# fabrizioromanelli/ORBSLAM2

Hardware: AMD Instinct MI355X
Metric: frames/sec ORB extract+match, KITTI 1241×376 stereo, 2000 feats; 1/2/4/8 GPU (higher is better)
Workload: dtype u8; 1 GPU; Stereo-KITTI00-02 1241x376, 2000 features, 8 levels: extract L+R + ComputeStereoMatches (64 pairs per step per GPU, weak scaling); distinct_pairs=16, chains_in_flight=1, stream_groups=1, quadtree_kernel=3, parallelism=frame-pair sharding, no data-path collective

## Files before the change

orbslam2_amd/csrc/orbfe_common.hpp:

```cpp
#pragma once

#include "orbfe_device.h"
#include <cstdlib>

typedef short pk16 __attribute__((ext_vector_type(2)));
#define ORBFE_RSRC_FLAGS 0x00020000

__device__ __forceinline__ int lane_id() { return threadIdx.x & 63; }

__device__ __forceinline__ int row_sum_i32(int v)
{
    v += __builtin_amdgcn_update_dpp(0, v, 0xB1, 0xf, 0xf, true);
    v += __builtin_amdgcn_update_dpp(0, v, 0x4E, 0xf, 0xf, true);
    v += __builtin_amdgcn_update_dpp(0, v, 0x141, 0xf, 0xf, true);
    v += __builtin_amdgcn_update_dpp(0, v, 0x140, 0xf, 0xf, true);
    return v;
}
__device__ __forceinline__ int wave_sum_i32(int v)
{
    v = row_sum_i32(v);
    v += __builtin_amdgcn_update_dpp(0, v, 0x142, 0xa, 0xf, false);
    v += __builtin_amdgcn_update_dpp(0, v, 0x143, 0xc, 0xf, false);
    return __builtin_amdgcn_readlane(v, 63);
}
__device__ __forceinline__ unsigned wave_min_u32(unsigned v)
{
#pragma unroll
    for (int o = 32; o > 0; o >>= 1) {
        unsigned t = (unsigned)__shfl_xor((int)v, o, 64);
        v = t < v ? t : v;
    }
    return v;
}

__host__ __device__ __forceinline__ int xcd_split_log2(int n_units) { return n_units >= 5 ? 0 : n_units >= 3 ? 1 : n_units == 2 ? 2 : 3; }
__host__ __forceinline__ int xcd_grid(int blocks_per_unit, int n_units)
{
    const int lg = xcd_split_log2(n_units), per_xcd = (blocks_per_unit + (1 << lg) - 1) >> lg, side = 8 >> lg;
    return per_xcd * ((n_units + side - 1) / side) * 8;
}
__device__ __forceinline__ int small_div(int a, int b) { return (int)(((float)a + 0.5f) * __builtin_amdgcn_rcpf((float)b)); }
__device__ __forceinline__ bool xcd_map_of(int bid, int blocks_per_unit, int n_units, int &unit, int &blk);
__device__ __forceinline__ bool xcd_map(int blocks_per_unit, int n_units, int &unit, int &blk) { return xcd_map_of((int)blockIdx.x, blocks_per_unit, n_units, unit, blk); }
__device__ __forceinline__ bool xcd_map_of(int bid, int blocks_per_unit, int n_units, int &unit, int &blk)
{
    const int lg = xcd_split_log2(n_units), xcd = bid & 7, jb = bid >> 3;
    const int per_xcd = (blocks_per_unit + (1 << lg) - 1) >> lg;
    const int round = small_div(jb, per_xcd);
    unit = round * (8 >> lg) + (xcd >> lg);
    blk = ((jb - round * per_xcd) << lg) + (xcd & ((1 << lg) - 1));
    return unit < n_units && blk < blocks_per_unit;
}

__host__ __forceinline__ uint32_t xcd_map_magic_host(int blocks_per_unit, int n_units)
{
    const int lg = xcd_split_log2(n_units), per_xcd = (blocks_per_unit + (1 << lg) - 1) >> lg, side = 8 >> lg;
    const unsigned long long rounds = (unsigned long long)((n_units + side - 1) / side);
    if (per_xcd <= 1 || (unsigned long long)per_xcd * rounds * (unsigned long long)per_xcd >= (1ull << 32)) return 0u;
    return (uint32_t)(((1ull << 32) + (unsigned long long)per_xcd - 1ull) / (unsigned long long)per_xcd);
}
__device__ __forceinline__ bool xcd_map_of_magic(int bid, int blocks_per_unit, int n_units, uint32_t magic, int &unit, int &blk)
{
    if (magic == 0u) return xcd_map_of(bid, blocks_per_unit, n_units, unit, blk);
    const int lg = xcd_split_log2(n_units), xcd = bid & 7, jb = bid >> 3;
    const int per_xcd = (blocks_per_unit + (1 << lg) - 1) >> lg;
    const int round = (int)__builtin_amdgcn_readfirstlane((int)(((unsigned long long)(unsigned)jb * (unsigned long long)magic) >> 32));
    unit = round * (8 >> lg) + (xcd >> lg);
    blk = ((jb - round * per_xcd) << lg) + (xcd & ((1 << lg) - 1));
    return unit < n_units && blk < blocks_per_unit;
}

__device__ __forceinline__ bool xcd_map_magic(int blocks_per_unit, int n_units, uint32_t magic, int &unit, int &blk) { return xcd_map_of_magic((int)blockIdx.x, blocks_per_unit, n_units, magic, unit, blk); }

__device__ __forceinline__ int reflect101(int p, int len)
{
    if (len == 1) return 0;
    while (p < 0 || p >= len) {
        if (p < 0) p = -p;
        else p = 2 * len - 2 - p;
    }
    return p;
}

__device__ inline int block_excl_scan(const int *src, int *dst, int n, int *s_tmp)
{
    const int nt = blockDim.x, tid = threadIdx.x;
    const int per = (n + nt - 1) / nt;
    const int b = tid * per;
    const int e = (b + per < n) ? b + per : n;
    int sum = 0;
    for (int i = b; i < e; i++) sum += src[i];
    s_tmp[tid] = sum;
    __syncthreads();
    for (int off = 1; off < nt; off <<= 1) {
        int v = tid >= off ? s_tmp[tid - off] : 0;
        __syncthreads();
        s_tmp[tid] += v;
        __syncthreads();
    }
    const int total = s_tmp[nt - 1];
    int run = s_tmp[tid] - sum;
    for (int i = b; i < e; i++) {
        int v = src[i];
        dst[i] = run;
        run += v;
    }
    __syncthreads();
    return total;
}

__device__ __forceinline__ float fast_atan2_deg(float y, float x)
{
    const float p1 = __uint_as_float(0x4265226fu);
    const float p3 = __uint_as_float(0xc19556eeu);
    const float p5 = __uint_as_float(0x410e9fbfu);
    const float p7 = __uint_as_float(0xc0228ad9u);
    const float eps = 2.220446049250313e-16f;
    float ax = fabsf(x), ay = fabsf(y);
    float a, c, c2;
    if (ax >= ay) {
        c = __fdiv_rn(ay, __fadd_rn(ax, eps));
        c2 = __fmul_rn(c, c);
        a = __fmul_rn(__fadd_rn(__fmul_rn(__fadd_rn(__fmul_rn(__fadd_rn(__fmul_rn(p7, c2), p5), c2), p3), c2), p1), c);
    } else {
        c = __fdiv_rn(ax, __fadd_rn(ay, eps));
        c2 = __fmul_rn(c, c);
        a = __fsub_rn(90.f, __fmul_rn(__fadd_rn(__fmul_rn(__fadd_rn(__fmul_rn(__fadd_rn(__fmul_rn(p7, c2), p5), c2), p3), c2), p1), c));
    }
    if (x < 0) a = __fsub_rn(180.f, a);
    if (y < 0) a = __fsub_rn(360.f, a);
    return a;
}

__device__ __forceinline__ void sincos_det(float rad, float *s, float *c)
{
    const double TWO_OVER_PI = 6.36619772367581382433e-01;
    const double PIO2_HI = 1.57079632673412561417e+00;
    const double PIO2_LO = 6.07710050650619224932e-11;
    const double S1 = -1.66666666666666324348e-01, S2 = 8.33333333332248946124e-03,
                 S3 = -1.98412698298579493134e-04, S4 = 2.75573137070700676789e-06,
                 S5 = -2.50507602534068634195e-08, S6 = 1.58969099521155010221e-10;
    const double C1 = 4.16666666666666019037e-02, C2 = -1.38888888888741095749e-03,
                 C3 = 2.48015872894767294178e-05, C4 = -2.75573143513906633035e-07,
                 C5 = 2.08757232129817482790e-09, C6 = -1.13596475577881948265e-11;
    double x = (double)rad;
    double t = __dadd_rn(__dmul_rn(x, TWO_OVER_PI), 0.5);
    int q = (int)t;
    if (t < 0.0 && (double)q != t) q -= 1;
    double qd = (double)q;
    double r = __dsub_rn(__dsub_rn(x, __dmul_rn(qd, PIO2_HI)), __dmul_rn(qd, PIO2_LO));
    double z = __dmul_rn(r, r);
    double sp = __dadd_rn(S2, __dmul_rn(z, __dadd_rn(S3, __dmul_rn(z, __dadd_rn(S4, __dmul_rn(z, __dadd_rn(S5, __dmul_rn(z, S6))))))));
    double sr = __dadd_rn(r, __dmul_rn(__dmul_rn(z, r), __dadd_rn(S1, __dmul_rn(z, sp))));
    double cp = __dmul_rn(z, __dadd_rn(C1, __dmul_rn(z, __dadd_rn(C2, __dmul_rn(z, __dadd_rn(C3, __dmul_rn(z, __dadd_rn(C4, __dmul_rn(z, __dadd_rn(C5, __dmul_rn(z, C6)))))))))));
    double cr = __dsub_rn(1.0, __dsub_rn(__dmul_rn(0.5, z), __dmul_rn(z, cp)));
    double sv, cv;
    switch (q & 3) {
    case 0: sv = sr; cv = cr; break;
    case 1: sv = cr; cv = -sr; break;
    case 2: sv = -sr; cv = -cr; break;
    default: sv = -cr; cv = sr; break;
    }
    *s = (float)sv;
    *c = (float)cv;
}

__device__ __forceinline__ int hamming256(const uint32_t *a, const uint32_t *b)
{
    int d = 0;
#pragma unroll
    for (int i = 0; i < 8; i++) d += __popc(a[i] ^ b[i]);
    return d;
}

__device__ __forceinline__ const uint8_t *level_image(const DeviceConfig &cfg, const DeviceBuffers &buf, int img, int level, int &pitch)
{
    if (level == 0) { pitch = buf.lv0_pitch; return buf.lv0 + (size_t)img * buf.lv0_stride; }
    const LevelInfo &L = cfg.lv[level];
    pitch = L.pitch;
    return buf.pyr + (size_t)img * cfg.pyr_bytes + L.pyr_off;
}

struct __attribute__((packed, aligned(4))) orbfe_u4_unaligned { uint32_t x, y, z, w; };
__device__ __forceinline__ uint4 load16_unaligned(const uint8_t *p)
{
    const orbfe_u4_unaligned t = *(const orbfe_u4_unaligned *)p;
    return make_uint4(t.x, t.y, t.z, t.w);
}

struct __attribute__((packed, aligned(1))) orbfe_u4_any { uint32_t x, y, z, w; };
__device__ __forceinline__ uint4 load16_any(const uint8_t *p)
{
    const orbfe_u4_any t = *(const orbfe_u4_any *)p;
    return make_uint4(t.x, t.y, t.z, t.w);
}

struct __attribute__((packed, aligned(4))) orbfe_u3_unaligned { uint32_t x, y, z; };

typedef uint32_t orbfe_u32x4 __attribute__((ext_vector_type(4)));
__device__ __forceinline__ uint32_t const_load_u32(const uint32_t *p) { return *(const __attribute__((address_space(4))) uint32_t *)(uintptr_t)p; }
__device__ __forceinline__ uint4 const_load_u32x4(const uint4 *p)
{
    const orbfe_u32x4 v = *(const __attribute__((address_space(4))) orbfe_u32x4 *)(uintptr_t)p;
    return make_uint4(v.x, v.y, v.z, v.w);
}
```

orbslam2_amd/csrc/orbfe_stereo.hip:

```cpp
#include "orbfe_common.hpp"


#define SM_G 16
#define SM_WIN_BYTES (11 * 16 + 11 * 32 + 16)
__device__ __forceinline__ unsigned group_min_u32(unsigned v)
{
#pragma unroll
    for (int o = SM_G / 2; o > 0; o >>= 1) {
        const unsigned t = (unsigned)__shfl_xor((int)v, o, 64);
        v = t < v ? t : v;
    }
    return v;
}
__device__ __forceinline__ int group_sum_i32(int v) { return row_sum_i32(v); }
__device__ __forceinline__ uint32_t sad_u16(uint32_t a, uint32_t b, uint32_t c) { uint32_t d; asm("v_sad_u16 %0, %1, %2, %3" : "=v"(d) : "v"(a), "v"(b), "v"(c)); return d; }

#include "orbfe_rowlist.hpp"

__global__ __launch_bounds__(256) void stereo_rowlist_kernel(DeviceConfig cfg, DeviceBuffers buf)
{
    extern __shared__ __attribute__((aligned(16))) uint8_t s_rl_all[];
    const int wave = __builtin_amdgcn_readfirstlane((int)(threadIdx.x >> 6));
    rowlist_wave<RL_ROWS_ALONE>(cfg, buf, blockIdx.y, (int)blockIdx.x * 4 + wave, s_rl_all + wave * RL_LDS_BYTES);
}

__global__ __launch_bounds__(256) void stereo_match_kernel(DeviceConfig cfg, DeviceBuffers buf, int n_pairs)
{
    __shared__ uint2 s_cand[(256 / SM_G) * 4 * SM_G];
    __shared__ __attribute__((aligned(16))) uint8_t s_win[(256 / SM_G) * SM_WIN_BYTES];
    const int kpb = 256 / SM_G;
    const int bpp = (cfg.sel_total + kpb - 1) / kpb;
    int pair, blk;
    if (!xcd_map_magic(bpp, n_pairs, cfg.xcd_magic, pair, blk)) return;
    const int imgL = 2 * pair, imgR = 2 * pair + 1;
    const int gl = threadIdx.x & (SM_G - 1);
    const int iL = blk * kpb + (threadIdx.x / SM_G);
    const int nL = buf.kp_cnt[imgL], nR = buf.kp_cnt[imgR];
    if (iL >= nL) return;
    const KeyPointPOD *kL = (const KeyPointPOD *)buf.kps + (size_t)imgL * cfg.sel_total;
    const KeyPointPOD *kR = (const KeyPointPOD *)buf.kps + (size_t)imgR * cfg.sel_total;
    const uint8_t *dL = buf.desc + (size_t)imgL * cfg.sel_total * 32;
    const uint8_t *dR = buf.desc + (size_t)imgR * cfg.sel_total * 32;
    float *u_right = buf.u_right + (size_t)imgL * cfg.sel_total;
    float *depth = buf.depth + (size_t)imgL * cfg.sel_total;
    int *sad_out = buf.sad + (size_t)imgL * cfg.sel_total;

    const KeyPointPOD kp = kL[iL];
    const int level_l = kp.octave;
    const float uL = kp.x, vL = kp.y;
    const int row = (int)vL;
    const float min_z = cfg.mb;
    const float max_d = __fdiv_rn(cfg.bf, min_z);
    const float min_u = __fsub_rn(uL, max_d);
    const float max_u = uL;

    uint32_t dl[8];
    {
        const uint4 *p = (const uint4 *)(dL + (size_t)iL * 32);
        const uint4 lo = p[0], hi = p[1];
        dl[0] = lo.x; dl[1] = lo.y; dl[2] = lo.z; dl[3] = lo.w; dl[4] = hi.x; dl[5] = hi.y; dl[6] = hi.z; dl[7] = hi.w;
    }
    unsigned best = (100u << 16) | 0xffffu;
    float best_x = 0.f;
    auto consider = [&](int iR, int oct, float xr) {
        if (oct >= level_l - 1 && oct <= level_l + 1 && xr >= min_u && xr <= max_u) {
            const uint4 *p = (const uint4 *)(dR + (size_t)iR * 32);
            const uint4 lo = p[0], hi = p[1];
            const uint32_t dr[8] = {lo.x, lo.y, lo.z, lo.w, hi.x, hi.y, hi.z, hi.w};
            const unsigned key = ((unsigned)hamming256(dl, dr) << 16) | (unsigned)iR;
            if (key < best) { best = key; best_x = xr; }
        }
    };
    int cnt = 0;
    if (row >= 0 && row < cfg.height) cnt = buf.row_cnt[(size_t)pair * cfg.height + row];
    if (cnt <= cfg.row_cap) {
        const uint2 *rent = buf.row_ent + ((size_t)pair * cfg.height + row) * cfg.row_cap;
        uint2 *s_list = s_cand + (threadIdx.x / SM_G) * (4 * SM_G);
        const int gshift = (threadIdx.x & 63) & ~(SM_G - 1);
        for (int j0 = 0; j0 < cnt; j0 += 4 * SM_G) {
            uint2 e[4];
            bool ok[4];
#pragma unroll
            for (int u = 0; u < 4; u++) {
                const int j = j0 + gl + SM_G * u;
                e[u] = rent[j < cnt ? j : cnt - 1];
            }
            int n_pass = 0;
#pragma unroll
            for (int u = 0; u < 4; u++) {
                const int j = j0 + gl + SM_G * u;
                const int oct = (int)(e[u].x >> 16);
                const float xr = __uint_as_float(e[u].y);
                ok[u] = j < cnt && oct >= level_l - 1 && oct <= level_l + 1 && xr >= min_u && xr <= max_u;
                const unsigned slice = (unsigned)(__ballot(ok[u]) >> gshift) & ((1u << SM_G) - 1u);
                if (ok[u]) s_list[n_pass + __popc(slice & ((1u << gl) - 1u))] = e[u];
                n_pass += __popc(slice);
            }
            __builtin_amdgcn_s_waitcnt(0xc07f);
            __builtin_amdgcn_wave_barrier();
            for (int k = gl; k < n_pass; k += SM_G) {
                const uint2 c = s_list[k];
                const int iR = (int)(c.x & 0xffffu);
                const uint4 *p = (const uint4 *)(dR + (size_t)iR * 32);
                const uint4 lo = p[0], hi = p[1];
                const uint32_t dr[8] = {lo.x, lo.y, lo.z, lo.w, hi.x, hi.y, hi.z, hi.w};
                const unsigned key = ((unsigned)hamming256(dl, dr) << 16) | (unsigned)iR;
                if (key < best) { best = key; best_x = __uint_as_float(c.y); }
            }
            __builtin_amdgcn_s_waitcnt(0xc07f);
            __builtin_amdgcn_wave_barrier();
        }
    } else {
        for (int iR = gl; iR < nR; iR += SM_G) {
            const KeyPointPOD kr = kR[iR];
            const float r = __fmul_rn(2.0f, cfg.lv[kr.octave].scale);
            const int maxr = (int)ceilf(__fadd_rn(kr.y, r));
            const int minr = (int)floorf(__fsub_rn(kr.y, r));
            if (row >= minr && row <= maxr) consider(iR, kr.octave, kr.x);
        }
    }
    const unsigned gbest = group_min_u32(best);
    const int best_dist = (int)(gbest >> 16);
    float uR0 = best == gbest ? best_x : 0.f;
    {
        int bits = __float_as_int(uR0);
#pragma unroll
        for (int o = SM_G / 2; o > 0; o >>= 1) bits |= __shfl_xor(bits, o, 64);
        uR0 = __int_as_float(bits);
    }
    float out_u = -1.0f, out_d = -1.0f;
    int out_sad = -1;
    if (best_dist < 75) {
        const float sf = cfg.lv[level_l].inv_scale;
        const float s_uL = roundf(__fmul_rn(kp.x, sf));
        const float s_vL = roundf(__fmul_rn(kp.y, sf));
        const float s_uR0 = roundf(__fmul_rn(uR0, sf));
        const LevelInfo &L = cfg.lv[level_l];
        const int cu = (int)s_uL, cv = (int)s_vL, cr = (int)s_uR0;
        const float iniu = s_uR0;
        const float endu = __fadd_rn(s_uR0, 11.0f);
        const bool in_ref = !(iniu < 0 || endu >= (float)L.w);
        const bool safe = cu - 5 >= 0 && cu + 5 < L.w && cv - 5 >= 0 && cv + 5 < L.h && cr - 10 >= 0 && cr + 10 < L.w;
        if (in_ref && safe) {
            int lpitch;
            const uint8_t *imL = level_image(cfg, buf, imgL, level_l, lpitch);
            const uint8_t *imR = level_image(cfg, buf, imgR, level_l, lpitch);
            uint8_t *wl = s_win + (threadIdx.x / SM_G) * SM_WIN_BYTES, *wr = wl + 11 * 16;
            if (gl < 11) {
                const unsigned ro = (unsigned)__mul24(cv - 5 + gl, lpitch);
                const uint4 a = load16_unaligned(imL + ro + cu - 5);
                const uint4 b0 = load16_unaligned(imR + ro + cr - 10), b1 = load16_unaligned(imR + ro + cr + 6);
                *(uint4 *)(wl + 16 * gl) = a;
                *(uint4 *)(wr + 32 * gl) = b0;
                *(uint4 *)(wr + 32 * gl + 16) = b1;
            }
            __builtin_amdgcn_s_waitcnt(0xc07f);
            __builtin_amdgcn_wave_barrier();
            auto window = [&](int row, int o, uint32_t (&w)[3]) {
                const uint32_t *q = (const uint32_t *)(wr + 32 * row + (o & ~3));
                const uint32_t q0 = q[0], q1 = q[1], q2 = q[2], q3 = q[3];
                const unsigned sh = (unsigned)(o & 3);
                w[0] = __builtin_amdgcn_alignbyte(q1, q0, sh); w[1] = __builtin_amdgcn_alignbyte(q2, q1, sh); w[2] = __builtin_amdgcn_alignbyte(q3, q2, sh);
            };
            const int lc = wl[16 * 5 + 5];
            uint32_t rcw[3];
            window(5, 5, rcw);
            const uint32_t lc2 = (uint32_t)lc * 0x10001u;
            uint32_t rc2[11], acc[11];
#pragma unroll
            for (int i = 0; i < 11; i++) {
                const uint32_t word = rcw[i >> 2];
                const uint32_t sel = (i & 3) == 0 ? 0x0c000c00u : ((i & 3) == 1 ? 0x0c010c01u : ((i & 3) == 2 ? 0x0c020c02u : 0x0c030c03u));
                rc2[i] = __builtin_amdgcn_perm(0u, word, sel);
                acc[i] = 0u;
            }
#pragma unroll
            for (int t = 0; t < 8; t += 2) {
                const int p0 = gl + SM_G * t, p1 = p0 + SM_G;
                const int py0 = (p0 * 745) >> 13, px0 = p0 - py0 * 11;
                const int p1c = p1 < 121 ? p1 : p0;
                const int py1 = (p1c * 745) >> 13, px1 = p1c - py1 * 11;
                const uint32_t il2 = (uint32_t)wl[16 * py0 + px0] | ((uint32_t)wl[16 * py1 + px1] << 16);
                uint32_t w0[3], w1[3];
                window(py0, px0, w0);
                window(py1, px1, w1);
                const uint32_t m = p1 < 121 ? 0xffffffffu : 0x0000ffffu;
#pragma unroll
                for (int i = 0; i < 11; i++) {
                    const uint32_t sel = (i & 3) == 0 ? 0x0c040c00u : ((i & 3) == 1 ? 0x0c050c01u : ((i & 3) == 2 ? 0x0c060c02u : 0x0c070c03u));
                    const uint32_t ir2 = __builtin_amdgcn_perm(w1[i >> 2], w0[i >> 2], sel);
                    uint32_t x2 = il2 + rc2[i], y2 = ir2 + lc2;
                    if (t == 6) { x2 &= m; y2 &= m; }
                    acc[i] = sad_u16(x2, y2, acc[i]);
                }
            }
            int dists[11];
#pragma unroll
            for (int i = 0; i < 11; i++) dists[i] = (int)acc[i];
            int sad_best = 0x7fffffff, best_inc = 0;
#pragma unroll
            for (int i = 0; i < 11; i++) {
                dists[i] = group_sum_i32(dists[i]);
                if (dists[i] < sad_best) { sad_best = dists[i]; best_inc = i - 5; }
            }
            out_sad = -2 - sad_best;
            if (best_inc != -5 && best_inc != 5) {
                float d1 = 0.f, d2 = 0.f, d3 = 0.f;
#pragma unroll
                for (int t = 1; t < 10; t++)
                    if (t == best_inc + 5) { d1 = (float)dists[t - 1]; d2 = (float)dists[t]; d3 = (float)dists[t + 1]; }
                const float delta = __fdiv_rn(__fsub_rn(d1, d3), __fmul_rn(2.0f, __fsub_rn(__fadd_rn(d1, d3), __fmul_rn(2.0f, d2))));
                if (!(delta < -1.0f || delta > 1.0f)) {
                    float best_ur = __fmul_rn(L.scale, __fadd_rn(__fadd_rn(s_uR0, (float)best_inc), delta));
                    float disparity = __fsub_rn(uL, best_ur);
                    if (disparity >= 0.0f && disparity < max_d) {
                        if (disparity <= 0.0f) {
                            disparity = 0.01f;
                            best_ur = (float)__dsub_rn((double)uL, 0.01);
                        }
                        out_d = __fdiv_rn(cfg.bf, disparity);
                        out_u = best_ur;
                        out_sad = sad_best;
                    }
                }
            }
        }
    }
    if (gl == 0) {
        u_right[iL] = out_u;
        depth[iL] = out_d;
        sad_out[iL] = out_sad;
    }
}

__global__ __launch_bounds__(256) void stereo_median_kernel(DeviceConfig cfg, DeviceBuffers buf)
{
    extern __shared__ int s_vals[];
    __shared__ int s_hist[256];
    __shared__ int s_sel[3];
    const int pair = blockIdx.x;
    const int imgL = 2 * pair;
    const int tid = threadIdx.x, lane = tid & 63;
    const int nL = buf.kp_cnt[imgL];
    float *u_right = buf.u_right + (size_t)imgL * cfg.sel_total;
    float *depth = buf.depth + (size_t)imgL * cfg.sel_total;
    const int *sad = buf.sad + (size_t)imgL * cfg.sel_total;
    for (int i = tid; i < nL; i += 256) s_vals[i] = sad[i];
    unsigned prefix = 0, mask = 0;
    for (int shift = 8; shift >= 0; shift -= 8) {
        s_hist[tid] = 0;
        __syncthreads();
        for (int i = tid; i < nL; i += 256) {
            const int v = s_vals[i];
            if (v >= 0 && ((unsigned)v & mask) == prefix) atomicAdd(&s_hist[((unsigned)v >> shift) & 255u], 1);
        }
        __syncthreads();
        if (tid < 64) {
            const int h0 = s_hist[4 * lane], h1 = s_hist[4 * lane + 1], h2 = s_hist[4 * lane + 2], h3 = s_hist[4 * lane + 3];
            const int sum = h0 + h1 + h2 + h3;
            int inc = sum;
#pragma unroll
            for (int o = 1; o < 64; o <<= 1) {
                const int t = __shfl_up(inc, o, 64);
                if (lane >= o) inc += t;
            }
            const int total = __shfl(inc, 63, 64);
            if (shift == 8 && lane == 0) s_sel[2] = total;
            const int rank = shift == 8 ? total / 2 : s_sel[1];
            const int before = inc - sum;
            if (total > 0 && rank >= before && rank < inc) {
                int r = rank - before, d = 4 * lane;
                if (r >= h0) { r -= h0; d++; if (r >= h1) { r -= h1; d++; if (r >= h2) { r -= h2; d++; } } }
                s_sel[0] = d;
                s_sel[1] = r;
            }
        }
        __syncthreads();
        if (s_sel[2] == 0) return;
        prefix |= (unsigned)s_sel[0] << shift;
        mask |= 255u << shift;
        __syncthreads();
    }
    const float median = (float)(int)prefix;
    const float th_dist = __fmul_rn(__fmul_rn(1.5f, 1.4f), median);
    for (int i = tid; i < nL; i += 256) {
        const int v = s_vals[i];
        if (v >= 0 && !((float)v < th_dist)) { u_right[i] = -1.0f; depth[i] = -1.0f; }
    }
}

__device__ inline void undistort_point(const DeviceConfig &cfg, float uf, float vf, float &uo, float &vo)
{
    if (cfg.n_dist == 0 || cfg.dist[0] == 0.0f) { uo = uf; vo = vf; return; }
    const double k0 = cfg.dist[0], k1 = cfg.dist[1], k2 = cfg.dist[2], k3 = cfg.dist[3], k4 = cfg.n_dist > 4 ? (double)cfg.dist[4] : 0.0;
    const double fx = cfg.cam[0], fy = cfg.cam[1], cx = cfg.cam[2], cy = cfg.cam[3], ifx = 1. / fx, ify = 1. / fy;
    const double u = uf, v = vf;
    double x = (u - cx) * ifx, y = (v - cy) * ify;
    const double x0 = x, y0 = y;
    for (int j = 0; j < 5; j++) {
        const double r2 = x * x + y * y;
        const double icdist = (1 + ((0.0 * r2 + 0.0) * r2 + 0.0) * r2) / (1 + ((k4 * r2 + k1) * r2 + k0) * r2);
        if (icdist < 0) { x = (u - cx) * ifx; y = (v - cy) * ify; break; }
        const double deltaX = 2 * k2 * x * y + k3 * (r2 + 2 * x * x) + 0.0 * r2 + 0.0 * r2 * r2;
        const double deltaY = k2 * (r2 + 2 * y * y) + 2 * k3 * x * y + 0.0 * r2 + 0.0 * r2 * r2;
        x = (x0 - deltaX) * icdist;
        y = (y0 - deltaY) * icdist;
    }
    const double xx = fx * x + 0.0 * y + cx, yy = 0.0 * x + fy * y + cy, ww = 1. / (0.0 * x + 0.0 * y + 1.0);
    uo = (float)(xx * ww);
    vo = (float)(yy * ww);
}

__global__ __launch_bounds__(256) void undistort_kernel(DeviceConfig cfg, const KeyPointPOD *__restrict__ in, KeyPointPOD *__restrict__ out, int n)
{
    const int i = blockIdx.x * 256 + threadIdx.x;
    if (i >= n) return;
    KeyPointPOD kp = in[i];
    undistort_point(cfg, kp.x, kp.y, kp.x, kp.y);
    out[i] = kp;
}

void orbfe_launch_undistort(const DeviceConfig &cfg, const void *d_keys_in, void *d_keys_out, int n, hipStream_t s)
{
    if (n > 0) hipLaunchKernelGGL(undistort_kernel, dim3((n + 255) / 256), dim3(256), 0, s, cfg, (const KeyPointPOD *)d_keys_in, (KeyPointPOD *)d_keys_out, n);
}

template <typename T>
__global__ __launch_bounds__(256) void rgbd_kernel(DeviceConfig cfg, DeviceBuffers buf, const T *__restrict__ depth_img,
                                                   size_t pitch_floats, int img, float factor)
{
    const int i = blockIdx.x * 256 + threadIdx.x;
    img += (int)blockIdx.y;
    depth_img += (size_t)blockIdx.y * pitch_floats * (size_t)cfg.height;
    const int n = buf.kp_cnt[img];
    if (i >= n) return;
    const KeyPointPOD kp = ((const KeyPointPOD *)buf.kps)[(size_t)img * cfg.sel_total + i];
    float u = -1.0f, dp = -1.0f;
    const int v = (int)kp.y, uu = (int)kp.x;
    if (uu >= 0 && v >= 0 && uu < cfg.width && v < cfg.height) {
        float d;
        if constexpr (sizeof(T) == 2) d = __fmul_rn((float)depth_img[(size_t)v * pitch_floats + uu], factor);
        else d = depth_img[(size_t)v * pitch_floats + uu];
        if (d > 0) {
            float xu, yu;
            undistort_point(cfg, kp.x, kp.y, xu, yu);
            dp = d;
            u = __fsub_rn(xu, __fdiv_rn(cfg.bf, d));
        }
    }
    buf.u_right[(size_t)img * cfg.sel_total + i] = u;
    buf.depth[(size_t)img * cfg.sel_total + i] = dp;
}

__global__ __launch_bounds__(256) void hamming_matrix_kernel(const uint8_t *__restrict__ da, int na,
                                                             const uint8_t *__restrict__ db, int nb, int *__restrict__ dist)
{
    const int j = blockIdx.x * 64 + (threadIdx.x & 63);
    const int i0 = (blockIdx.y * 4 + (threadIdx.x >> 6)) * 16;
    if (j >= nb) return;
    uint32_t b[8];
    const uint32_t *pb = (const uint32_t *)(db + (size_t)j * 32);
#pragma unroll
    for (int k = 0; k < 8; k++) b[k] = pb[k];
    for (int i = i0; i < i0 + 16 && i < na; i++) {
        const uint32_t *pa = (const uint32_t *)(da + (size_t)i * 32);
        uint32_t a[8];
#pragma unroll
        for (int k = 0; k < 8; k++) a[k] = pa[k];
        dist[(size_t)i * nb + j] = hamming256(a, b);
    }
}


void orbfe_launch_stereo_rowlists(const DeviceConfig &cfg, const DeviceBuffers &buf, int n_pairs, hipStream_t s)
{
    dim3 grid((rowlist_blocks(cfg.height, RL_ROWS_ALONE) + 3) / 4, n_pairs);
    hipLaunchKernelGGL(stereo_rowlist_kernel, grid, dim3(256), 4 * RL_LDS_BYTES, s, cfg, buf);
}

void orbfe_launch_stereo_match(const DeviceConfig &cfg_in, const DeviceBuffers &buf, int n_pairs, hipStream_t s)
{
    const int kpb = 256 / SM_G;
    DeviceConfig cfg = cfg_in;
    cfg.xcd_magic = xcd_map_magic_host((cfg.sel_total + kpb - 1) / kpb, n_pairs);
    dim3 grid(xcd_grid((cfg.sel_total + kpb - 1) / kpb, n_pairs));
    hipLaunchKernelGGL(stereo_match_kernel, grid, dim3(256), 0, s, cfg, buf, n_pairs);
}

void orbfe_launch_stereo_median(const DeviceConfig &cfg, const DeviceBuffers &buf, int n_pairs, hipStream_t s)
{
    hipLaunchKernelGGL(stereo_median_kernel, dim3(n_pairs), dim3(256), (size_t)cfg.sel_total * sizeof(int), s, cfg, buf);
}

void orbfe_launch_rgbd(const DeviceConfig &cfg, const DeviceBuffers &buf, const float *d_depth, size_t depth_pitch_floats,
                       int image, hipStream_t s)
{
    hipLaunchKernelGGL(rgbd_kernel<float>, dim3((cfg.sel_total + 255) / 256), dim3(256), 0, s, cfg, buf, d_depth, depth_pitch_floats, image, 1.0f);
}

void orbfe_launch_rgbd_u16(const DeviceConfig &cfg, const DeviceBuffers &buf, const uint16_t *d_depth, size_t depth_pitch_px,
                           float factor, int image, hipStream_t s)
{
    hipLaunchKernelGGL(rgbd_kernel<uint16_t>, dim3((cfg.sel_total + 255) / 256), dim3(256), 0, s, cfg, buf, d_depth, depth_pitch_px, image, factor);
}

void orbfe_launch_rgbd_batch(const DeviceConfig &cfg, const DeviceBuffers &buf, const void *d_depth, bool is_u16, float factor, int n_images, hipStream_t s)
{
    dim3 grid((cfg.sel_total + 255) / 256, n_images);
    if (is_u16) hipLaunchKernelGGL(rgbd_kernel<uint16_t>, grid, dim3(256), 0, s, cfg, buf, (const uint16_t *)d_depth, (size_t)cfg.width, 0, factor);
    else hipLaunchKernelGGL(rgbd_kernel<float>, grid, dim3(256), 0, s, cfg, buf, (const float *)d_depth, (size_t)cfg.width, 0, 1.0f);
}

__global__ __launch_bounds__(256) void pack_results_kernel(DeviceConfig cfg, DeviceBuffers buf, uint8_t *__restrict__ out, PackedOffsets lay, int img_step, int stereo)
{
    const int oi = blockIdx.y, di = oi * img_step;
    const int cap = cfg.sel_total, j0 = (int)blockIdx.x * 256, j = j0 + (int)threadIdx.x;
    const int n = buf.kp_cnt[di];
    const int *lc = buf.sel_cnt + (size_t)di * cfg.nlevels;
    if (blockIdx.x == 0 && threadIdx.x == 0) {
        ((int *)(out + lay.counts))[oi] = n;
        for (int l = 0; l < cfg.nlevels; l++) ((int *)(out + lay.level_counts))[oi * cfg.nlevels + l] = lc[l];
    }
    if (j < n) {
        int l = 0, first = 0;
        for (; l < cfg.nlevels - 1; l++) {
            const int c = lc[l];
            if (j < first + c) break;
            first += c;
        }
        const int slot = cfg.lv[l].sel_off + (j - first);
        const unsigned mb = (unsigned)cfg.min_border * 0x10001u;
        ((uint32_t *)(out + lay.xy))[(size_t)oi * cap + j] = buf.sel_xy[(size_t)di * cap + slot] + mb;
        ((float *)(out + lay.angle))[(size_t)oi * cap + j] = ((const KeyPointPOD *)buf.kps)[(size_t)di * cap + j].angle;
        (out + lay.response)[(size_t)oi * cap + j] = buf.sel_sc[(size_t)di * cap + slot];
    }
    {
        const uint4 *src = (const uint4 *)(buf.desc + ((size_t)di * cap + j0) * 32);
        uint4 *dst = (uint4 *)(out + lay.desc + ((size_t)oi * cap + j0) * 32);
        const int chunks = 2 * (cap - j0 < 256 ? cap - j0 : 256);
        for (int c = threadIdx.x; c < chunks; c += 256) dst[c] = src[c];
    }
    if (stereo && (di & 1) == 0 && j < cap) {
        const int pr = di >> 1;
        ((float *)(out + lay.u_right))[(size_t)pr * cap + j] = buf.u_right[(size_t)di * cap + j];
        ((float *)(out + lay.depth))[(size_t)pr * cap + j] = buf.depth[(size_t)di * cap + j];
    }
}

void orbfe_launch_pack_results(const DeviceConfig &cfg, const DeviceBuffers &buf, uint8_t *d_out, const PackedOffsets &lay, int n_out, int img_step, bool stereo, hipStream_t s)
{
    dim3 grid((cfg.sel_total + 255) / 256, n_out);
    hipLaunchKernelGGL(pack_results_kernel, grid, dim3(256), 0, s, cfg, buf, d_out, lay, img_step, stereo ? 1 : 0);
}

void orbfe_launch_hamming_matrix(const uint8_t *da, int na, const uint8_t *db, int nb, int *dist, hipStream_t s)
{
    dim3 grid((nb + 63) / 64, (na + 63) / 64);
    hipLaunchKernelGGL(hamming_matrix_kernel, grid, dim3(256), 0, s, da, na, db, nb, dist);
}
```

Before: 100,600 frames/s (1 frame = 1 stereo pair).

## Compact SAD refinement jobs across block groups and compute windows in registers

The stereo match kernel now runs in two phases. First each 16-lane group does the descriptor search, and keypoints that pass the SAD-window checks write a job record to shared memory. After a block barrier, the surviving jobs are compacted onto the first groups, which do the 11x11 SAD refinement. The SAD windows now live in registers and are shared with shuffles and byte permutes instead of a shared-memory staging buffer, and the first row-list loads are issued before the count is read. This cuts divergence and idle groups in the SAD phase and LDS traffic, at the cost of an extra __syncthreads and more register pressure.

```diff
diff --git a/orbslam2_amd/csrc/orbfe_common.hpp b/orbslam2_amd/csrc/orbfe_common.hpp
--- a/orbslam2_amd/csrc/orbfe_common.hpp
+++ b/orbslam2_amd/csrc/orbfe_common.hpp
@@ -173,12 +173,17 @@
     return d;
 }
 
+__device__ __forceinline__ const uint8_t *level_image_at(const DeviceConfig &cfg, const DeviceBuffers &buf, int img, int level, int lv_pitch, int lv_pyr_off, int &pitch)
+{
+    if (level == 0) { pitch = buf.lv0_pitch; return buf.lv0 + (size_t)img * buf.lv0_stride; }
+    pitch = lv_pitch;
+    return buf.pyr + (size_t)img * cfg.pyr_bytes + lv_pyr_off;
+}
 __device__ __forceinline__ const uint8_t *level_image(const DeviceConfig &cfg, const DeviceBuffers &buf, int img, int level, int &pitch)
 {
     if (level == 0) { pitch = buf.lv0_pitch; return buf.lv0 + (size_t)img * buf.lv0_stride; }
     const LevelInfo &L = cfg.lv[level];
-    pitch = L.pitch;
-    return buf.pyr + (size_t)img * cfg.pyr_bytes + L.pyr_off;
+    return level_image_at(cfg, buf, img, level, L.pitch, L.pyr_off, pitch);
 }
 
 struct __attribute__((packed, aligned(4))) orbfe_u4_unaligned { uint32_t x, y, z, w; };
diff --git a/orbslam2_amd/csrc/orbfe_stereo.hip b/orbslam2_amd/csrc/orbfe_stereo.hip
--- a/orbslam2_amd/csrc/orbfe_stereo.hip
+++ b/orbslam2_amd/csrc/orbfe_stereo.hip
@@ -2,7 +2,8 @@
 
 
 #define SM_G 16
-#define SM_WIN_BYTES (11 * 16 + 11 * 32 + 16)
+#define SM_GROUPS (256 / SM_G)
+#define SM_K SM_GROUPS
 __device__ __forceinline__ unsigned group_min_u32(unsigned v)
 {
 #pragma unroll
@@ -26,17 +27,16 @@
 
 __global__ __launch_bounds__(256) void stereo_match_kernel(DeviceConfig cfg, DeviceBuffers buf, int n_pairs)
 {
-    __shared__ uint2 s_cand[(256 / SM_G) * 4 * SM_G];
-    __shared__ __attribute__((aligned(16))) uint8_t s_win[(256 / SM_G) * SM_WIN_BYTES];
-    const int kpb = 256 / SM_G;
-    const int bpp = (cfg.sel_total + kpb - 1) / kpb;
+    __shared__ uint2 s_cand[SM_GROUPS * 4 * SM_G];
+    __shared__ uint4 s_job[SM_GROUPS][2];
+    __shared__ int s_njob[4];
+    const int bpp = (cfg.sel_total + SM_K - 1) / SM_K;
     int pair, blk;
     if (!xcd_map_magic(bpp, n_pairs, cfg.xcd_magic, pair, blk)) return;
     const int imgL = 2 * pair, imgR = 2 * pair + 1;
-    const int gl = threadIdx.x & (SM_G - 1);
-    const int iL = blk * kpb + (threadIdx.x / SM_G);
+    const int gl = threadIdx.x & (SM_G - 1), grp = threadIdx.x / SM_G;
+    const int lane = threadIdx.x & 63, wave = threadIdx.x >> 6;
     const int nL = buf.kp_cnt[imgL], nR = buf.kp_cnt[imgR];
-    if (iL >= nL) return;
     const KeyPointPOD *kL = (const KeyPointPOD *)buf.kps + (size_t)imgL * cfg.sel_total;
     const KeyPointPOD *kR = (const KeyPointPOD *)buf.kps + (size_t)imgR * cfg.sel_total;
     const uint8_t *dL = buf.desc + (size_t)imgL * cfg.sel_total * 32;
@@ -44,192 +44,220 @@
     float *u_right = buf.u_right + (size_t)imgL * cfg.sel_total;
     float *depth = buf.depth + (size_t)imgL * cfg.sel_total;
     int *sad_out = buf.sad + (size_t)imgL * cfg.sel_total;
-
-    const KeyPointPOD kp = kL[iL];
-    const int level_l = kp.octave;
-    const float uL = kp.x, vL = kp.y;
-    const int row = (int)vL;
     const float min_z = cfg.mb;
     const float max_d = __fdiv_rn(cfg.bf, min_z);
-    const float min_u = __fsub_rn(uL, max_d);
-    const float max_u = uL;
-
-    uint32_t dl[8];
+
+    int wave_jobs;
     {
-        const uint4 *p = (const uint4 *)(dL + (size_t)iL * 32);
-        const uint4 lo = p[0], hi = p[1];
-        dl[0] = lo.x; dl[1] = lo.y; dl[2] = lo.z; dl[3] = lo.w; dl[4] = hi.x; dl[5] = hi.y; dl[6] = hi.z; dl[7] = hi.w;
-    }
-    unsigned best = (100u << 16) | 0xffffu;
-    float best_x = 0.f;
-    auto consider = [&](int iR, int oct, float xr) {
-        if (oct >= level_l - 1 && oct <= level_l + 1 && xr >= min_u && xr <= max_u) {
-            const uint4 *p = (const uint4 *)(dR + (size_t)iR * 32);
+        const int iL = blk * SM_K + grp;
+        const KeyPointPOD kp = kL[iL];
+        const bool valid = iL < nL;
+        const int level_l = valid ? kp.octave : 0;
+        const float uL = kp.x, vL = kp.y;
+        const int row = (int)vL;
+        const LevelInfo &L = cfg.lv[level_l];
+        const int lv_w = L.w, lv_h = L.h, lv_pitch = L.pitch, lv_off = L.pyr_off;
+        const float lv_scale = L.scale, sf = L.inv_scale;
+        const float min_u = __fsub_rn(uL, max_d);
+        const float max_u = uL;
+
+        uint32_t dl[8];
+        {
+            const uint4 *p = (const uint4 *)(dL + (size_t)iL * 32);
             const uint4 lo = p[0], hi = p[1];
-            const uint32_t dr[8] = {lo.x, lo.y, lo.z, lo.w, hi.x, hi.y, hi.z, hi.w};
-            const unsigned key = ((unsigned)hamming256(dl, dr) << 16) | (unsigned)iR;
-            if (key < best) { best = key; best_x = xr; }
-        }
-    };
-    int cnt = 0;
-    if (row >= 0 && row < cfg.height) cnt = buf.row_cnt[(size_t)pair * cfg.height + row];
-    if (cnt <= cfg.row_cap) {
-        const uint2 *rent = buf.row_ent + ((size_t)pair * cfg.height + row) * cfg.row_cap;
-        uint2 *s_list = s_cand + (threadIdx.x / SM_G) * (4 * SM_G);
-        const int gshift = (threadIdx.x & 63) & ~(SM_G - 1);
-        for (int j0 = 0; j0 < cnt; j0 += 4 * SM_G) {
-            uint2 e[4];
-            bool ok[4];
-#pragma unroll
-            for (int u = 0; u < 4; u++) {
-                const int j = j0 + gl + SM_G * u;
-                e[u] = rent[j < cnt ? j : cnt - 1];
-            }
-            int n_pass = 0;
-#pragma unroll
-            for (int u = 0; u < 4; u++) {
-                const int j = j0 + gl + SM_G * u;
-                const int oct = (int)(e[u].x >> 16);
-                const float xr = __uint_as_float(e[u].y);
-                ok[u] = j < cnt && oct >= level_l - 1 && oct <= level_l + 1 && xr >= min_u && xr <= max_u;
-                const unsigned slice = (unsigned)(__ballot(ok[u]) >> gshift) & ((1u << SM_G) - 1u);
-                if (ok[u]) s_list[n_pass + __popc(slice & ((1u << gl) - 1u))] = e[u];
-                n_pass += __popc(slice);
-            }
-            __builtin_amdgcn_s_waitcnt(0xc07f);
-            __builtin_amdgcn_wave_barrier();
-            for (int k = gl; k < n_pass; k += SM_G) {
-                const uint2 c = s_list[k];
-                const int iR = (int)(c.x & 0xffffu);
+            dl[0] = lo.x; dl[1] = lo.y; dl[2] = lo.z; dl[3] = lo.w; dl[4] = hi.x; dl[5] = hi.y; dl[6] = hi.z; dl[7] = hi.w;
+        }
+        unsigned best = (100u << 16) | 0xffffu;
+        float best_x = 0.f;
+        auto consider = [&](int iR, int oct, float xr) {
+            if (oct >= level_l - 1 && oct <= level_l + 1 && xr >= min_u && xr <= max_u) {
                 const uint4 *p = (const uint4 *)(dR + (size_t)iR * 32);
                 const uint4 lo = p[0], hi = p[1];
                 const uint32_t dr[8] = {lo.x, lo.y, lo.z, lo.w, hi.x, hi.y, hi.z, hi.w};
                 const unsigned key = ((unsigned)hamming256(dl, dr) << 16) | (unsigned)iR;
-                if (key < best) { best = key; best_x = __uint_as_float(c.y); }
-            }
-            __builtin_amdgcn_s_waitcnt(0xc07f);
-            __builtin_amdgcn_wave_barrier();
-        }
-    } else {
-        for (int iR = gl; iR < nR; iR += SM_G) {
-            const KeyPointPOD kr = kR[iR];
-            const float r = __fmul_rn(2.0f, cfg.lv[kr.octave].scale);
-            const int maxr = (int)ceilf(__fadd_rn(kr.y, r));
-            const int minr = (int)floorf(__fsub_rn(kr.y, r));
-            if (row >= minr && row <= maxr) consider(iR, kr.octave, kr.x);
-        }
-    }
-    const unsigned gbest = group_min_u32(best);
-    const int best_dist = (int)(gbest >> 16);
-    float uR0 = best == gbest ? best_x : 0.f;
-    {
-        int bits = __float_as_int(uR0);
-#pragma unroll
-        for (int o = SM_G / 2; o > 0; o >>= 1) bits |= __shfl_xor(bits, o, 64);
-        uR0 = __int_as_float(bits);
-    }
-    float out_u = -1.0f, out_d = -1.0f;
-    int out_sad = -1;
-    if (best_dist < 75) {
-        const float sf = cfg.lv[level_l].inv_scale;
-        const float s_uL = roundf(__fmul_rn(kp.x, sf));
-        const float s_vL = roundf(__fmul_rn(kp.y, sf));
-        const float s_uR0 = roundf(__fmul_rn(uR0, sf));
-        const LevelInfo &L = cfg.lv[level_l];
-        const int cu = (int)s_uL, cv = (int)s_vL, cr = (int)s_uR0;
-        const float iniu = s_uR0;
-        const float endu = __fadd_rn(s_uR0, 11.0f);
-        const bool in_ref = !(iniu < 0 || endu >= (float)L.w);
-        const bool safe = cu - 5 >= 0 && cu + 5 < L.w && cv - 5 >= 0 && cv + 5 < L.h && cr - 10 >= 0 && cr + 10 < L.w;
-        if (in_ref && safe) {
-            int lpitch;
-            const uint8_t *imL = level_image(cfg, buf, imgL, level_l, lpitch);
-            const uint8_t *imR = level_image(cfg, buf, imgR, level_l, lpitch);
-            uint8_t *wl = s_win + (threadIdx.x / SM_G) * SM_WIN_BYTES, *wr = wl + 11 * 16;
-            if (gl < 11) {
-                const unsigned ro = (unsigned)__mul24(cv - 5 + gl, lpitch);
-                const uint4 a = load16_unaligned(imL + ro + cu - 5);
-                const uint4 b0 = load16_unaligned(imR + ro + cr - 10), b1 = load16_unaligned(imR + ro + cr + 6);
-                *(uint4 *)(wl + 16 * gl) = a;
-                *(uint4 *)(wr + 32 * gl) = b0;
-                *(uint4 *)(wr + 32 * gl + 16) = b1;
-            }
-            __builtin_amdgcn_s_waitcnt(0xc07f);
-            __builtin_amdgcn_wave_barrier();
-            auto window = [&](int row, int o, uint32_t (&w)[3]) {
-                const uint32_t *q = (const uint32_t *)(wr + 32 * row + (o & ~3));
-                const uint32_t q0 = q[0], q1 = q[1], q2 = q[2], q3 = q[3];
-                const unsigned sh = (unsigned)(o & 3);
-                w[0] = __builtin_amdgcn_alignbyte(q1, q0, sh); w[1] = __builtin_amdgcn_alignbyte(q2, q1, sh); w[2] = __builtin_amdgcn_alignbyte(q3, q2, sh);
-            };
-            const int lc = wl[16 * 5 + 5];
-            uint32_t rcw[3];
-            window(5, 5, rcw);
-            const uint32_t lc2 = (uint32_t)lc * 0x10001u;
-            uint32_t rc2[11], acc[11];
-#pragma unroll
-            for (int i = 0; i < 11; i++) {
-                const uint32_t word = rcw[i >> 2];
-                const uint32_t sel = (i & 3) == 0 ? 0x0c000c00u : ((i & 3) == 1 ? 0x0c010c01u : ((i & 3) == 2 ? 0x0c020c02u : 0x0c030c03u));
-                rc2[i] = __builtin_amdgcn_perm(0u, word, sel);
-                acc[i] = 0u;
-            }
-#pragma unroll
-            for (int t = 0; t < 8; t += 2) {
-                const int p0 = gl + SM_G * t, p1 = p0 + SM_G;
-                const int py0 = (p0 * 745) >> 13, px0 = p0 - py0 * 11;
-                const int p1c = p1 < 121 ? p1 : p0;
-                const int py1 = (p1c * 745) >> 13, px1 = p1c - py1 * 11;
-                const uint32_t il2 = (uint32_t)wl[16 * py0 + px0] | ((uint32_t)wl[16 * py1 + px1] << 16);
-                uint32_t w0[3], w1[3];
-                window(py0, px0, w0);
-                window(py1, px1, w1);
-                const uint32_t m = p1 < 121 ? 0xffffffffu : 0x0000ffffu;
-#pragma unroll
-                for (int i = 0; i < 11; i++) {
-                    const uint32_t sel = (i & 3) == 0 ? 0x0c040c00u : ((i & 3) == 1 ? 0x0c050c01u : ((i & 3) == 2 ? 0x0c060c02u : 0x0c070c03u));
-                    const uint32_t ir2 = __builtin_amdgcn_perm(w1[i >> 2], w0[i >> 2], sel);
-                    uint32_t x2 = il2 + rc2[i], y2 = ir2 + lc2;
-                    if (t == 6) { x2 &= m; y2 &= m; }
-                    acc[i] = sad_u16(x2, y2, acc[i]);
-                }
-            }
-            int dists[11];
-#pragma unroll
-            for (int i = 0; i < 11; i++) dists[i] = (int)acc[i];
-            int sad_best = 0x7fffffff, best_inc = 0;
-#pragma unroll
-            for (int i = 0; i < 11; i++) {
-                dists[i] = group_sum_i32(dists[i]);
-                if (dists[i] < sad_best) { sad_best = dists[i]; best_inc = i - 5; }
-            }
-            out_sad = -2 - sad_best;
-            if (best_inc != -5 && best_inc != 5) {
-                float d1 = 0.f, d2 = 0.f, d3 = 0.f;
-#pragma unroll
-                for (int t = 1; t < 10; t++)
-                    if (t == best_inc + 5) { d1 = (float)dists[t - 1]; d2 = (float)dists[t]; d3 = (float)dists[t + 1]; }
-                const float delta = __fdiv_rn(__fsub_rn(d1, d3), __fmul_rn(2.0f, __fsub_rn(__fadd_rn(d1, d3), __fmul_rn(2.0f, d2))));
-                if (!(delta < -1.0f || delta > 1.0f)) {
-                    float best_ur = __fmul_rn(L.scale, __fadd_rn(__fadd_rn(s_uR0, (float)best_inc), delta));
-                    float disparity = __fsub_rn(uL, best_ur);
-                    if (disparity >= 0.0f && disparity < max_d) {
-                        if (disparity <= 0.0f) {
-                            disparity = 0.01f;
-                            best_ur = (float)__dsub_rn((double)uL, 0.01);
-                        }
-                        out_d = __fdiv_rn(cfg.bf, disparity);
-                        out_u = best_ur;
-                        out_sad = sad_best;
+                if (key < best) { best = key; best_x = xr; }
+            }
+        };
+        const bool row_ok = valid && row >= 0 && row < cfg.height;
+        const uint2 *rent = buf.row_ent + ((size_t)pair * cfg.height + (row_ok ? row : 0)) * cfg.row_cap;
+        uint2 e[4];
+#pragma unroll
+        for (int u = 0; u < 4; u++) {
+            const int j = gl + SM_G * u;
+            e[u] = rent[j < cfg.row_cap ? j : cfg.row_cap - 1];
+        }
+        int cnt = 0;
+        if (row_ok) cnt = buf.row_cnt[(size_t)pair * cfg.height + row];
+        if (cnt <= cfg.row_cap) {
+            uint2 *s_list = s_cand + grp * (4 * SM_G);
+            const int gshift = lane & ~(SM_G - 1);
+            for (int j0 = 0; j0 < cnt; j0 += 4 * SM_G) {
+                bool ok[4];
+                if (j0 > 0) {
+#pragma unroll
+                    for (int u = 0; u < 4; u++) {
+                        const int j = j0 + gl + SM_G * u;
+                        e[u] = rent[j < cnt ? j : cnt - 1];
                     }
                 }
-            }
-        }
-    }
-    if (gl == 0) {
-        u_right[iL] = out_u;
-        depth[iL] = out_d;
-        sad_out[iL] = out_sad;
+                int n_pass = 0;
+#pragma unroll
+                for (int u = 0; u < 4; u++) {
+                    const int j = j0 + gl + SM_G * u;
+                    const int oct = (int)(e[u].x >> 16);
+                    const float xr = __uint_as_float(e[u].y);
+                    ok[u] = j < cnt && oct >= level_l - 1 && oct <= level_l + 1 && xr >= min_u && xr <= max_u;
+                    const unsigned slice = (unsigned)(__ballot(ok[u]) >> gshift) & ((1u << SM_G) - 1u);
+                    if (ok[u]) s_list[n_pass + __popc(slice & ((1u << gl) - 1u))] = e[u];
+                    n_pass += __popc(slice);
+                }
+                __builtin_amdgcn_s_waitcnt(0xc07f);
+                __builtin_amdgcn_wave_barrier();
+                for (int k = gl; k < n_pass; k += SM_G) {
+                    const uint2 c = s_list[k];
+                    const int iR = (int)(c.x & 0xffffu);
+                    const uint4 *p = (const uint4 *)(dR + (size_t)iR * 32);
+                    const uint4 lo = p[0], hi = p[1];
+                    const uint32_t dr[8] = {lo.x, lo.y, lo.z, lo.w, hi.x, hi.y, hi.z, hi.w};
+                    const unsigned key = ((unsigned)hamming256(dl, dr) << 16) | (unsigned)iR;
+                    if (key < best) { best = key; best_x = __uint_as_float(c.y); }
+                }
+                __builtin_amdgcn_s_waitcnt(0xc07f);
+                __builtin_amdgcn_wave_barrier();
+            }
+        } else {
+            for (int iR = gl; iR < nR; iR += SM_G) {
+                const KeyPointPOD kr = kR[iR];
+                const float r = __fmul_rn(2.0f, cfg.lv[kr.octave].scale);
+                const int maxr = (int)ceilf(__fadd_rn(kr.y, r));
+                const int minr = (int)floorf(__fsub_rn(kr.y, r));
+                if (row >= minr && row <= maxr) consider(iR, kr.octave, kr.x);
+            }
+        }
+        const unsigned gbest = group_min_u32(best);
+        const int best_dist = (int)(gbest >> 16);
+        float uR0 = best == gbest ? best_x : 0.f;
+        {
+            int bits = __float_as_int(uR0);
+#pragma unroll
+            for (int o = SM_G / 2; o > 0; o >>= 1) bits |= __shfl_xor(bits, o, 64);
+            uR0 = __int_as_float(bits);
+        }
+        bool reach = false;
+        int cu = 0, cv = 0, cr = 0;
+        if (best_dist < 75) {
+            const float s_uL = roundf(__fmul_rn(kp.x, sf));
+            const float s_vL = roundf(__fmul_rn(kp.y, sf));
+            const float s_uR0 = roundf(__fmul_rn(uR0, sf));
+            cu = (int)s_uL; cv = (int)s_vL; cr = (int)s_uR0;
+            const float iniu = s_uR0;
+            const float endu = __fadd_rn(s_uR0, 11.0f);
+            const bool in_ref = !(iniu < 0 || endu >= (float)lv_w);
+            const bool safe = cu - 5 >= 0 && cu + 5 < lv_w && cv - 5 >= 0 && cv + 5 < lv_h && cr - 10 >= 0 && cr + 10 < lv_w;
+            reach = in_ref && safe;
+        }
+        const unsigned long long heads = __ballot(reach && gl == 0);
+        if (gl == 0) {
+            if (reach) {
+                uint4 *rec = s_job[wave * 4 + __popcll(heads & ((1ull << lane) - 1ull))];
+                int lpitch;
+                const uint8_t *imL = level_image_at(cfg, buf, imgL, level_l, lv_pitch, lv_off, lpitch);
+                const uint8_t *imR = level_image_at(cfg, buf, imgR, level_l, lv_pitch, lv_off, lpitch);
+                const unsigned ro = (unsigned)__mul24(cv - 5, lpitch);
+                const uint64_t pl = (uint64_t)(uintptr_t)(imL + ro + cu - 5), pr = (uint64_t)(uintptr_t)(imR + ro + cr - 10);
+                rec[0] = make_uint4((unsigned)iL | ((unsigned)cr << 16), (unsigned)lpitch, __float_as_uint(lv_scale), __float_as_uint(uL));
+                rec[1] = make_uint4((unsigned)pl, (unsigned)(pl >> 32), (unsigned)pr, (unsigned)(pr >> 32));
+            } else if (valid) {
+                u_right[iL] = -1.0f;
+                depth[iL] = -1.0f;
+                sad_out[iL] = -1;
+            }
+        }
+        wave_jobs = __popcll(heads);
+    }
+    if (lane == 0) s_njob[wave] = wave_jobs;
+    __syncthreads();
+
+    const int c0 = s_njob[0], c1 = s_njob[1], c2 = s_njob[2], c3 = s_njob[3];
+    const int n_jobs = c0 + c1 + c2 + c3;
+    if (grp < n_jobs) {
+        int seg = 0, k = grp;
+        if (k >= c0) { k -= c0; seg = 1; if (k >= c1) { k -= c1; seg = 2; if (k >= c2) { k -= c2; seg = 3; } } }
+        const uint4 job = s_job[seg * 4 + k][0], win = s_job[seg * 4 + k][1];
+        const int iL = (int)(job.x & 0xffffu);
+        const float uL = __uint_as_float(job.w), s_uR0 = (float)(job.x >> 16);
+        const uint8_t *pL = (const uint8_t *)(uintptr_t)((uint64_t)win.x | ((uint64_t)win.y << 32));
+        const uint8_t *pR = (const uint8_t *)(uintptr_t)((uint64_t)win.z | ((uint64_t)win.w << 32));
+        uint32_t lw[3] = {0u, 0u, 0u}, rw[6] = {0u, 0u, 0u, 0u, 0u, 0u};
+        if (gl < 11) {
+            const unsigned ro = (unsigned)__mul24(gl, (int)job.y);
+            const uint4 a = load16_unaligned(pL + ro);
+            const uint4 b0 = load16_unaligned(pR + ro), b1 = load16_unaligned(pR + ro + 16);
+            lw[0] = a.x; lw[1] = a.y; lw[2] = a.z;
+            rw[0] = b0.x; rw[1] = b0.y; rw[2] = b0.z; rw[3] = b0.w; rw[4] = b1.x; rw[5] = b1.y;
+        }
+        const uint32_t clw = (uint32_t)__shfl((int)lw[1], 5, SM_G);
+        const uint32_t crw[4] = {0u, (uint32_t)__shfl((int)rw[1], 5, SM_G), (uint32_t)__shfl((int)rw[2], 5, SM_G), (uint32_t)__shfl((int)rw[3], 5, SM_G)};
+        const uint32_t lc2 = __builtin_amdgcn_perm(0u, clw, 0x0c010c01u);
+        uint32_t rc2[11], acc[11], A[6], B[21];
+#pragma unroll
+        for (int i = 0; i < 11; i++) {
+            const uint32_t o = (uint32_t)((i + 5) & 3);
+            rc2[i] = __builtin_amdgcn_perm(0u, crw[(i + 5) >> 2], 0x0c000c00u | o | (o << 16));
+            acc[i] = 0u;
+        }
+#pragma unroll
+        for (int k = 0; k < 6; k++) {
+            const uint32_t o = (uint32_t)((2 * k) & 3);
+            A[k] = __builtin_amdgcn_perm(0u, lw[(2 * k) >> 2], k < 5 ? (0x0c000c00u | o | ((o + 1u) << 16)) : (0x0c0c0c00u | o));
+        }
+#pragma unroll
+        for (int j = 0; j < 21; j++) {
+            const uint32_t o = (uint32_t)(j & 3);
+            B[j] = __builtin_amdgcn_perm(rw[(j >> 2) + (j < 20 ? 1 : 0)], rw[j >> 2], 0x0c000c00u | o | ((o + 1u) << 16)) + lc2;
+        }
+#pragma unroll
+        for (int i = 0; i < 11; i++) {
+#pragma unroll
+            for (int k = 0; k < 5; k++) acc[i] = sad_u16(A[k] + rc2[i], B[2 * k + i], acc[i]);
+            acc[i] = sad_u16(A[5] + rc2[i], __builtin_amdgcn_perm(rc2[i], B[10 + i], 0x07060100u), acc[i]);
+        }
+        int dists[11];
+#pragma unroll
+        for (int i = 0; i < 11; i++) dists[i] = gl < 11 ? (int)acc[i] : 0;
+        int sad_best = 0x7fffffff, best_inc = 0;
+#pragma unroll
+        for (int i = 0; i < 11; i++) {
+            dists[i] = group_sum_i32(dists[i]);
+            if (dists[i] < sad_best) { sad_best = dists[i]; best_inc = i - 5; }
+        }
+        float out_u = -1.0f, out_d = -1.0f;
+        int out_sad = -2 - sad_best;
+        if (best_inc != -5 && best_inc != 5) {
+            float d1 = 0.f, d2 = 0.f, d3 = 0.f;
+#pragma unroll
+            for (int t = 1; t < 10; t++)
+                if (t == best_inc + 5) { d1 = (float)dists[t - 1]; d2 = (float)dists[t]; d3 = (float)dists[t + 1]; }
+            const float delta = __fdiv_rn(__fsub_rn(d1, d3), __fmul_rn(2.0f, __fsub_rn(__fadd_rn(d1, d3), __fmul_rn(2.0f, d2))));
+            if (!(delta < -1.0f || delta > 1.0f)) {
+                float best_ur = __fmul_rn(__uint_as_float(job.z), __fadd_rn(__fadd_rn(s_uR0, (float)best_inc), delta));
+                float disparity = __fsub_rn(uL, best_ur);
+                if (disparity >= 0.0f && disparity < max_d) {
+                    if (disparity <= 0.0f) {
+                        disparity = 0.01f;
+                        best_ur = (float)__dsub_rn((double)uL, 0.01);
+                    }
+                    out_d = __fdiv_rn(cfg.bf, disparity);
+                    out_u = best_ur;
+                    out_sad = sad_best;
+                }
+            }
+        }
+        if (gl == 0) {
+            u_right[iL] = out_u;
+            depth[iL] = out_d;
+            sad_out[iL] = out_sad;
+        }
     }
 }
 
@@ -380,7 +408,7 @@
 
 void orbfe_launch_stereo_match(const DeviceConfig &cfg_in, const DeviceBuffers &buf, int n_pairs, hipStream_t s)
 {
-    const int kpb = 256 / SM_G;
+    const int kpb = SM_K;
     DeviceConfig cfg = cfg_in;
     cfg.xcd_magic = xcd_map_magic_host((cfg.sel_total + kpb - 1) / kpb, n_pairs);
     dim3 grid(xcd_grid((cfg.sel_total + kpb - 1) / kpb, n_pairs));
```

Result: faster. 101,800 frames/s (1 frame = 1 stereo pair) (median of 6 runs) (+1.1%).
